# Lance0218/Pytorch-DistributedDataParallel-Training-Tricks

Measured on AMD Instinct MI355X. Metric: images/sec, higher is better.
Workload: dtype bf16; 1 GPU; model=Toy_Net, dataset=MNIST(synthetic), global_batch=1024, per_gpu_batch=1024, parallelism=dp1, optimizer=FusedSGD(momentum=0.9,nesterov)+Lookahead(k=10,a=0.5)

## Files before the change

### ddp_tricks_amd/ops/hip/bindings.cpp

```cpp
#include <torch/extension.h>

void multi_tensor_unscale(std::vector<at::Tensor> grads, at::Tensor found_inf,
                          double inv_scale,
                          c10::optional<at::Tensor> partials);
void multi_tensor_sqsum(std::vector<at::Tensor> tensors, at::Tensor partials);
void norm_finalize(at::Tensor partials, long n, double max_norm,
                   c10::optional<at::Tensor> found_inf, at::Tensor out,
                   c10::optional<at::Tensor> stats);
void multi_tensor_scale(std::vector<at::Tensor> tensors, at::Tensor coef,
                        c10::optional<at::Tensor> found_inf);
long mt_chunk_elems();
void fused_sgd(std::vector<at::Tensor> params, std::vector<at::Tensor> grads,
               std::vector<at::Tensor> bufs, double lr, double momentum,
               double wd, double nesterov, c10::optional<at::Tensor> found_inf,
               c10::optional<at::Tensor> grad_scale);
void fused_lookahead(std::vector<at::Tensor> fast, std::vector<at::Tensor> slow,
                     double alpha, c10::optional<at::Tensor> found_inf);
at::Tensor cast_to_bf16(at::Tensor x);
at::Tensor pad8_channels(at::Tensor x);
at::Tensor nhwc_flatten(at::Tensor x);
at::Tensor nhwc_unflatten(at::Tensor dy, long C, long H, long W);
std::vector<at::Tensor> pack_conv_weight(at::Tensor w, bool pad8,
                                         bool want_wt2);

// ... 42 lines not shown
                                           at::Tensor beta,
                                           at::Tensor running_mean,
                                           at::Tensor running_var,
                                           double momentum, double eps,
                                           c10::optional<at::Tensor> pre_stats);
std::vector<at::Tensor> bn_bwd_pool2(at::Tensor x, at::Tensor dy_pooled,
                                     at::Tensor gamma, at::Tensor save_mean,
                                     at::Tensor save_invstd, at::Tensor code);
at::Tensor bn_sync_local(at::Tensor x, c10::optional<at::Tensor> pre_stats);
std::vector<at::Tensor> bn_sync_fwd(at::Tensor x, at::Tensor gathered,
                                    at::Tensor gamma, at::Tensor beta,
                                    at::Tensor running_mean,
                                    at::Tensor running_var, double momentum,
                                    double eps, bool fuse_relu,
                                    c10::optional<at::Tensor> residual);
at::Tensor bn_sync_bwd_local(at::Tensor x, at::Tensor dy,
                             at::Tensor save_mean, at::Tensor save_invstd,
                             at::Tensor mask, bool fuse_relu);
std::vector<at::Tensor> bn_sync_bwd_dx(at::Tensor x, at::Tensor dy,
                                       at::Tensor gamma, at::Tensor save_mean,
                                       at::Tensor save_invstd, at::Tensor mask,
                                       bool fuse_relu, at::Tensor gathered,
                                       at::Tensor count, bool want_dresid);

at::Tensor gemm_tn(at::Tensor A, at::Tensor B, c10::optional<at::Tensor> bias,
                   bool out_f32);
at::Tensor transpose_bf16(at::Tensor x);
at::Tensor col_sum(at::Tensor x);
at::Tensor linear_fwd(at::Tensor x, at::Tensor w, c10::optional<at::Tensor> bias);
at::Tensor linear_dgrad(at::Tensor dy, at::Tensor w);
at::Tensor linear_wgrad(at::Tensor dy, at::Tensor x);

at::Tensor conv2d_fwd(at::Tensor x, at::Tensor w, c10::optional<at::Tensor> bias,
                      long stride, long pad);
std::vector<at::Tensor> conv2d_fwd_stats(at::Tensor x, at::Tensor w,
                                         c10::optional<at::Tensor> bias,
                                         long stride, long pad);
at::Tensor conv2d_dgrad(at::Tensor dy, at::Tensor wt2, long N, long C, long H,
                        long W, long R, long S, long stride, long pad,
                        c10::optional<at::Tensor> addend, long group);
std::tuple<std::string, long, long, long> conv2d_dgrad_plan(
    long N, long C, long H, long W, long Ko, long R, long S, long stride,
    long pad, long group);
std::vector<at::Tensor> conv2d_dgrad_bn(at::Tensor dy, at::Tensor wt2,
                                        long N, long C, long H, long W,
                                        long R, long S, long pad,
                                        at::Tensor bn_x, at::Tensor bn_mask,
                                        at::Tensor bn_mean,
                                        at::Tensor bn_invstd);
at::Tensor conv2d_wgrad(at::Tensor dy, at::Tensor x, long R, long S,
                        long stride, long pad);
std::vector<at::Tensor> conv2d_wgrad_bias(at::Tensor dy, at::Tensor x,
                                          long R, long S, long stride,
                                          long pad);
std::tuple<std::string, long, bool> conv2d_wgrad_plan(
    long N, long C, long H, long W, long Ko, long R, long S, long stride,
    long pad, bool want_bias);

std::vector<at::Tensor> batch_gather_aug(at::Tensor store, at::Tensor labels,
                                         at::Tensor index, at::Tensor lut,
                                         long pad, bool hflip, long seed,
                                         long epoch);
std::vector<at::Tensor> batch_gather_cutmix(at::Tensor store, at::Tensor labels,
                                            at::Tensor index, at::Tensor lut,
                                            long pad, bool hflip, long seed,
                                            long epoch, long prob_thresh);

void register_comm(py::module_& m);

PYBIND11_MODULE(TORCH_EXTENSION_NAME, m) {
    register_comm(m);
    m.def("multi_tensor_unscale", &multi_tensor_unscale,
          "fused unscale + inf check over grad tensors; with partials also "
// ... 71 lines not shown
    m.def("bn_bwd_pool2", &bn_bwd_pool2,
          py::arg("x"), py::arg("dy_pooled"), py::arg("gamma"),
          py::arg("save_mean"), py::arg("save_invstd"), py::arg("code"));
    m.def("bn_sync_local", &bn_sync_local,
          "SyncBatchNorm forward, rank-local half: [sum | sumsq | count] row",
          py::arg("x"), py::arg("pre_stats") = c10::nullopt);
    m.def("bn_sync_fwd", &bn_sync_fwd,
          "SyncBatchNorm forward, cross-rank half over gathered rows",
          py::arg("x"), py::arg("gathered"), py::arg("gamma"),
          py::arg("beta"), py::arg("running_mean"), py::arg("running_var"),
          py::arg("momentum"), py::arg("eps"), py::arg("fuse_relu") = false,
          py::arg("residual") = c10::nullopt);
    m.def("bn_sync_bwd_local", &bn_sync_bwd_local,
          "SyncBatchNorm backward, rank-local half: [dbeta | dgamma] row",
          py::arg("x"), py::arg("dy"), py::arg("save_mean"),
          py::arg("save_invstd"), py::arg("mask"),
          py::arg("fuse_relu") = false);
    m.def("bn_sync_bwd_dx", &bn_sync_bwd_dx,
          "SyncBatchNorm backward, cross-rank half over gathered rows",
          py::arg("x"), py::arg("dy"), py::arg("gamma"), py::arg("save_mean"),
          py::arg("save_invstd"), py::arg("mask"), py::arg("fuse_relu"),
          py::arg("gathered"), py::arg("count"),
          py::arg("want_dresid") = false);
    m.def("gemm_tn", &gemm_tn, py::arg("A"), py::arg("B"),
          py::arg("bias") = c10::nullopt, py::arg("out_f32") = false);
    m.def("transpose_bf16", &transpose_bf16);
    m.def("col_sum", &col_sum);
    m.def("linear_fwd", &linear_fwd, py::arg("x"), py::arg("w"),
          py::arg("bias") = c10::nullopt);
    m.def("linear_dgrad", &linear_dgrad);
    m.def("linear_wgrad", &linear_wgrad);
    m.def("conv2d_fwd", &conv2d_fwd, py::arg("x"), py::arg("w"),
          py::arg("bias") = c10::nullopt, py::arg("stride") = 1,
          py::arg("pad") = 0);
    m.def("conv2d_fwd_stats", &conv2d_fwd_stats, py::arg("x"), py::arg("w"),
          py::arg("bias") = c10::nullopt, py::arg("stride") = 1,
          py::arg("pad") = 0);
    m.def("conv2d_dgrad", &conv2d_dgrad,
          py::arg("dy"), py::arg("wt2"), py::arg("N"), py::arg("C"),
          py::arg("H"), py::arg("W"), py::arg("R"), py::arg("S"),
          py::arg("stride"), py::arg("pad"),
          py::arg("addend") = c10::nullopt, py::arg("group") = -1);
    m.def("conv2d_dgrad_plan", &conv2d_dgrad_plan,
          "(name, G, k_tiles_issued, k_tiles_raster) conv2d_dgrad would run "
          "for this shape; group -1 automatic, 0 raster, 32/64/128 forces "
          "that tap-uniform group size; launches nothing",
          py::arg("N"), py::arg("C"), py::arg("H"), py::arg("W"),
          py::arg("Ko"), py::arg("R"), py::arg("S"), py::arg("stride"),
          py::arg("pad"), py::arg("group") = -1);
    m.def("conv2d_dgrad_bn", &conv2d_dgrad_bn);
    m.def("conv2d_wgrad", &conv2d_wgrad);
    m.def("conv2d_wgrad_bias", &conv2d_wgrad_bias);
    m.def("conv2d_wgrad_plan", &conv2d_wgrad_plan,
          "(leaf name, split, fused_bias) conv2d_wgrad[_bias] would run for "
          "this shape under this process's DDPX_WGRAD_V; launches nothing",
          py::arg("N"), py::arg("C"), py::arg("H"), py::arg("W"),
          py::arg("Ko"), py::arg("R"), py::arg("S"), py::arg("stride"),
          py::arg("pad"), py::arg("want_bias"));
    m.def("batch_gather_aug", &batch_gather_aug,
          "uint8 HWC device store -> (bf16 channels_last batch, labels): "
          "gather by index + crop/flip + LUT normalise in one launch",
          py::arg("store"), py::arg("labels"), py::arg("index"),
          py::arg("lut"), py::arg("pad"), py::arg("hflip"), py::arg("seed"),
          py::arg("epoch"));
    m.def("batch_gather_cutmix", &batch_gather_cutmix,
          "batch_gather_aug with CutMix: (images, labels_a, labels_b, lam); "
          "prob_thresh is the apply probability in 1/65536",
          py::arg("store"), py::arg("labels"), py::arg("index"),
          py::arg("lut"), py::arg("pad"), py::arg("hflip"), py::arg("seed"),
          py::arg("epoch"), py::arg("prob_thresh"));
}
```

### ddp_tricks_amd/ops/hip/conv.hip

```cpp

#include <torch/extension.h>
#include <ATen/hip/HIPContext.h>
#include <climits>
#include <string>
#include <tuple>
#include "common.h"

typedef short bf16x8_t __attribute__((ext_vector_type(8)));

constexpr int CBM = 128, CBK = 64;

struct ConvShape {
    int N, H, W, C;
    int Ko, R, S;
    int P, Q;
    int stride, pad;
    FastDiv fdQ, fdP, fdW, fdH, fdC, fdS, fdKo;
    int cls_a, cls_b, nr, ns;
    int taps_r[4], taps_s[4];
    int off_r[4], off_s[4];
    int Hfull, Wfull;
    FastDiv fdNs;
    FastDiv fdGHW;
    int lgG;
};

static inline void init_fastdiv(ConvShape& cs) {
    cs.fdQ.init(cs.Q); cs.fdP.init(cs.P); cs.fdW.init(cs.W);
    cs.fdH.init(cs.H); cs.fdC.init(cs.C); cs.fdS.init(cs.S);
    cs.fdKo.init(cs.Ko);
    cs.fdGHW.init(1); cs.lgG = 0;
}

__host__ __device__ inline unsigned dgrad_tap_mask(
        int m_first, int m_last, int GHW, int lgG, int H, int W, int P, int Q,
        int R, int S, int pad) {
    const int g0 = m_first / GHW, g1 = m_last / GHW;
    int pix0 = 0, pix1 = H * W - 1;
    if (g0 == g1) {
        pix0 = (m_first - g0 * GHW) >> lgG;
        pix1 = (m_last - g0 * GHW) >> lgG;
    }
    const int h0 = pix0 / W, h1 = pix1 / W;
    unsigned mask = 0;
    for (int h = h0; h <= h1; ++h) {
        const int wa = h == h0 ? pix0 - h0 * W : 0;
        const int wb = h == h1 ? pix1 - h1 * W : W - 1;
        const int ra = h + pad - P + 1 > 0 ? h + pad - P + 1 : 0;
        const int rb = h + pad < R - 1 ? h + pad : R - 1;
        const int sa = wa + pad - Q + 1 > 0 ? wa + pad - Q + 1 : 0;
        const int sb = wb + pad < S - 1 ? wb + pad : S - 1;
        for (int r = ra; r <= rb; ++r)
            for (int sx = sa; sx <= sb; ++sx)
                mask |= 1u << (r * S + sx);
    }
    return mask;
}


__device__ __align__(16) unsigned char g_zero16[16];

struct BnFuse {
    const bf16* x;
    const unsigned char* mask;
    const float* mean;
    const float* invstd;
    float* slab;
};

template <int MODE, int TBN, int WAVES_M, int WAVES_N, bool STRIDE1,
          int CBM_T, bool TAPS = false>
__device__ __forceinline__
void conv_gemm_body(const bf16* __restrict__ Asrc,
                    const bf16* __restrict__ Bsrc,
                    const float* __restrict__ bias, bf16* __restrict__ out,
                    const ConvShape& cs, int M, int Kgemm, int Nout,
                    float* __restrict__ stats, BnFuse bn,
                    const bf16* __restrict__ addin) {
    constexpr int WM = CBM_T / WAVES_M;
    constexpr int WN = TBN / WAVES_N;
    constexpr int MI = WM / 16;
    constexpr int NI = WN / 16;
    constexpr int A_CHUNKS = CBM_T / 8;
    constexpr int B_CHUNKS = TBN / 8;
    __shared__ bf16 lds_a[1][CBM_T][CBK];
    __shared__ bf16 lds_b[1][TBN][CBK];
    static_assert(!TAPS || (MODE == 1 && STRIDE1), "TAPS is stride-1 dgrad");
    const int tile_m = TAPS && (gridDim.x & 7) == 0
        ? (int)(blockIdx.x & 7) * (int)(gridDim.x >> 3) + (int)(blockIdx.x >> 3)
        : (int)blockIdx.x;
    const int m0 = tile_m * CBM_T;
    const int n0 = blockIdx.y * TBN;
    const int tid = threadIdx.x;
    const int lane = tid & 63;
    const int wid = tid >> 6;
    const int wr = wid / WAVES_N, wc = wid % WAVES_N;

    f32x4 acc[MI][NI] = {};
    const int pl_row = lane >> 3;
    const int pl_segp = lane & 7;

    constexpr int A_PER = A_CHUNKS / 4;
    long ri_nb[A_PER];
    int ri_u[A_PER], ri_v[A_PER];
    #pragma unroll
    for (int ci = 0; ci < A_PER; ++ci) {
        const int ch = wid + ci * 4;
        const int row = ch * 8 + pl_row;
        const int gm = m0 + row;
        ri_u[ci] = INT_MIN;
        if (gm < M) {
            if (MODE == 0) {
                unsigned rem = fd_div(gm, cs.fdQ);
                int q = fd_mod(gm, cs.fdQ, rem);
                unsigned n = fd_div(rem, cs.fdP);
                int p = fd_mod(rem, cs.fdP, n);
                ri_nb[ci] = (long)n * cs.H;
                ri_u[ci] = p * cs.stride - cs.pad;
                ri_v[ci] = q * cs.stride - cs.pad;
            } else if (MODE == 2) {
                unsigned rem = fd_div(gm, cs.fdW);
                int w1 = fd_mod(gm, cs.fdW, rem);
                unsigned n = fd_div(rem, cs.fdH);
                int h1 = fd_mod(rem, cs.fdH, n);
                ri_nb[ci] = (long)n * cs.P;
                ri_u[ci] = h1;
                ri_v[ci] = w1;
            } else if (TAPS) {
                unsigned grp = fd_div(gm, cs.fdGHW);
                unsigned rem = fd_mod(gm, cs.fdGHW, grp);
                unsigned pix = rem >> cs.lgG;
                unsigned n = (grp << cs.lgG) + (rem & ((1u << cs.lgG) - 1));
                unsigned h = fd_div(pix, cs.fdW);
                int wcol = fd_mod(pix, cs.fdW, h);
                ri_nb[ci] = (long)n * cs.P;
                ri_u[ci] = (int)h + cs.pad;
                ri_v[ci] = wcol + cs.pad;
            } else {
                unsigned rem = fd_div(gm, cs.fdW);
                int wcol = fd_mod(gm, cs.fdW, rem);
                unsigned n = fd_div(rem, cs.fdH);
                int h = fd_mod(rem, cs.fdH, n);
                ri_nb[ci] = (long)n * cs.P;
                ri_u[ci] = h + cs.pad;
                ri_v[ci] = wcol + cs.pad;
            }
        }
    }

    auto issue_tile = [&](int kt, int buf) {
        #pragma unroll
        for (int ci = 0; ci < A_PER; ++ci) {
            const int ch = wid + ci * 4;
            int row = ch * 8 + pl_row;
            int seg = pl_segp ^ (row & 7);
            int gk = kt + seg * 8;
            const bf16* src = reinterpret_cast<const bf16*>(g_zero16);
            if (ri_u[ci] != INT_MIN && gk < Kgemm) {
                if (MODE == 0) {
                    unsigned rs = fd_div(gk, cs.fdC);
                    int c = fd_mod(gk, cs.fdC, rs);
                    int r = fd_div(rs, cs.fdS);
                    int sx = fd_mod(rs, cs.fdS, r);
                    int h = ri_u[ci] + r;
                    int wcol = ri_v[ci] + sx;
                    if (h >= 0 && h < cs.H && wcol >= 0 && wcol < cs.W)
                        src = &Asrc[((ri_nb[ci] + h) * cs.W + wcol) * cs.C + c];
                } else if (MODE == 2) {
                    unsigned rs2 = fd_div(gk, cs.fdKo);
                    int ko = fd_mod(gk, cs.fdKo, rs2);
                    int ti = fd_div(rs2, cs.fdNs);
                    int si = fd_mod(rs2, cs.fdNs, ti);
                    int p = ri_u[ci] + cs.off_r[ti];
                    int q = ri_v[ci] + cs.off_s[si];
                    if (p >= 0 && p < cs.P && q >= 0 && q < cs.Q)
                        src = &Asrc[((ri_nb[ci] + p) * cs.Q + q) * cs.Ko + ko];
                } else if (STRIDE1) {
                    unsigned rs = fd_div(gk, cs.fdKo);
                    int ko = fd_mod(gk, cs.fdKo, rs);
                    int r = fd_div(rs, cs.fdS);
                    int sx = fd_mod(rs, cs.fdS, r);
// ... 19 lines not shown
                (__attribute__((address_space(3))) unsigned short*)&lds_a[buf][ch * 8][0],
                16, 0, 0);
        }
        for (int ch = wid; ch < B_CHUNKS; ch += 4) {
            int row = ch * 8 + pl_row;
            int seg = pl_segp ^ (row & 7);
            int gn = n0 + row, gk = kt + seg * 8;
            const bf16* src = reinterpret_cast<const bf16*>(g_zero16);
            if (MODE == 2) {
                if (gn < Nout && gk < Kgemm) {
                    unsigned rs2 = fd_div(gk, cs.fdKo);
                    int ko = fd_mod(gk, cs.fdKo, rs2);
                    int ri = fd_div(rs2, cs.fdNs);
                    int si = fd_mod(rs2, cs.fdNs, ri);
                    long gk_full = ((long)cs.taps_r[ri] * cs.S
                                    + cs.taps_s[si]) * cs.Ko + ko;
                    src = &Bsrc[(long)gn * (cs.R * cs.S * cs.Ko) + gk_full];
                }
            } else if (gn < Nout && gk < Kgemm)
                src = &Bsrc[(long)gn * Kgemm + gk];
            __builtin_amdgcn_global_load_lds(
                (const __attribute__((address_space(1))) unsigned short*)src,
                (__attribute__((address_space(3))) unsigned short*)&lds_b[buf][ch * 8][0],
                16, 0, 0);
        }
    };

    constexpr int buf = 0;
    unsigned tap_mask = 0;
    if (TAPS)
        tap_mask = __builtin_amdgcn_readfirstlane(dgrad_tap_mask(
            m0, min(m0 + CBM_T, M) - 1, (int)cs.fdGHW.d, cs.lgG, cs.H, cs.W,
            cs.P, cs.Q, cs.R, cs.S, cs.pad));
    int tap = 0, tap_end = cs.Ko;
    for (int kt = 0; kt < Kgemm; kt += CBK) {
        if (TAPS) {
            if (kt == tap_end) { ++tap; tap_end += cs.Ko; }
            if (!((tap_mask >> tap) & 1u)) { kt = tap_end - CBK; continue; }
        }
        issue_tile(kt, 0);
        __syncthreads();
        #pragma unroll
        for (int ks = 0; ks < CBK; ks += 32) {
            bf16x8_t af[MI], bfr[NI];
            const int kgrp = (ks >> 3) + (lane >> 4);
            #pragma unroll
            for (int mi = 0; mi < MI; ++mi) {
                int row = wr * WM + mi * 16 + (lane & 15);
                af[mi] = *reinterpret_cast<const bf16x8_t*>(
                    &lds_a[buf][row][(kgrp ^ (row & 7)) * 8]);
            }
            #pragma unroll
            for (int ni = 0; ni < NI; ++ni) {
                int row = wc * WN + ni * 16 + (lane & 15);
                bfr[ni] = *reinterpret_cast<const bf16x8_t*>(
                    &lds_b[buf][row][(kgrp ^ (row & 7)) * 8]);
            }
            #pragma unroll
            for (int mi = 0; mi < MI; ++mi)
                #pragma unroll
                for (int ni = 0; ni < NI; ++ni)
                    acc[mi][ni] = __builtin_amdgcn_mfma_f32_16x16x32_bf16(
                        af[mi], bfr[ni], acc[mi][ni], 0, 0, 0);
        }
        __syncthreads();
    }

    float psum[NI] = {}, psq[NI] = {};
    #pragma unroll
    for (int mi = 0; mi < MI; ++mi)
        #pragma unroll
        for (int ni = 0; ni < NI; ++ni) {
            int col = n0 + wc * WN + ni * 16 + (lane & 15);
            if (col >= Nout) continue;
            float badd = bias ? bias[col] : 0.f;
            #pragma unroll
            for (int r = 0; r < 4; ++r) {
                int row = m0 + wr * WM + mi * 16 + (lane >> 4) * 4 + r;
                if (row >= M) continue;
                if (MODE == 0 && stats) {
                    float v = acc[mi][ni][r] + badd;
                    psum[ni] += v;
                    psq[ni] = fmaf(v, v, psq[ni]);
                }
                if (MODE == 2) {
                    unsigned rem = fd_div(row, cs.fdW);
                    int w1 = fd_mod(row, cs.fdW, rem);
                    unsigned n = fd_div(rem, cs.fdH);
                    int h1 = fd_mod(rem, cs.fdH, n);
                    long addr = (((long)n * cs.Hfull + cs.cls_a
                                  + (long)h1 * cs.stride) * cs.Wfull
                                 + cs.cls_b + (long)w1 * cs.stride) * Nout
                                + col;
                    out[addr] = f2bf(acc[mi][ni][r] + badd);
                }
            }
        }

// ... 106 lines not shown
        float* red = reinterpret_cast<float*>(&lds_a[0][0][0]);
        #pragma unroll
        for (int ni = 0; ni < NI; ++ni) {
            float a = psum[ni], b = psq[ni];
            a += __shfl_down(a, 32, 64);
            a += __shfl_down(a, 16, 64);
            b += __shfl_down(b, 32, 64);
            b += __shfl_down(b, 16, 64);
            if ((lane & 48) == 0) {
                int cl = wc * WN + ni * 16 + (lane & 15);
                red[(wr * TBN + cl) * 2] = a;
                red[(wr * TBN + cl) * 2 + 1] = b;
            }
        }
        __syncthreads();
        const int gridM = gridDim.x;
        for (int cl = tid; cl < TBN; cl += 256) {
            float a = 0.f, b = 0.f;
            #pragma unroll
            for (int w = 0; w < WAVES_M; ++w) {
                a += red[(w * TBN + cl) * 2];
                b += red[(w * TBN + cl) * 2 + 1];
            }
            int col = n0 + cl;
            if (col < Nout) {
                stats[(long)col * gridM + blockIdx.x] = a;
                stats[(long)Nout * gridM + (long)col * gridM + blockIdx.x] = b;
            }
        }
    }
}

template <int MODE, int TBN, int WAVES_M, int WAVES_N, bool STRIDE1 = true,
          int CBM_T = CBM, bool TAPS = false>
__global__ __launch_bounds__(256, 4)
void k_conv_gemm(const bf16* __restrict__ Asrc, const bf16* __restrict__ Bsrc,
                 const float* __restrict__ bias, bf16* __restrict__ out,
                 ConvShape cs, int M, int Kgemm, int Nout,
                 float* __restrict__ stats = nullptr,
                 BnFuse bn = BnFuse{},
                 const bf16* __restrict__ addin = nullptr) {
    conv_gemm_body<MODE, TBN, WAVES_M, WAVES_N, STRIDE1, CBM_T, TAPS>(
        Asrc, Bsrc, bias, out, cs, M, Kgemm, Nout, stats, bn, addin);
}


struct ClsPack {
    ConvShape cs[4];
    int M[4];
    int K[4];
};

template <int TBN, int WAVES_M, int WAVES_N>
__global__ __launch_bounds__(256, 4)
void k_conv_gemm_cls(const bf16* __restrict__ Asrc,
                     const bf16* __restrict__ Bsrc, bf16* __restrict__ out,
                     ClsPack pack, int Nout) {
    const int z = blockIdx.z;
    const int M = pack.M[z];
    if ((int)blockIdx.x * CBM >= M) return;
    conv_gemm_body<2, TBN, WAVES_M, WAVES_N, true, CBM>(
        Asrc, Bsrc, nullptr, out, pack.cs[z], M, pack.K[z], Nout,
        nullptr, BnFuse{}, nullptr);
}

__global__ void k_conv_small_cin(const bf16* __restrict__ x,
                                 const bf16* __restrict__ w,
                                 const float* __restrict__ bias,
                                 bf16* __restrict__ y, ConvShape cs, long M) {
    extern __shared__ __attribute__((aligned(16))) char smem[];
    bf16* wlds = reinterpret_cast<bf16*>(smem);
    int rsc = cs.R * cs.S * cs.C;
    for (int i = threadIdx.x; i < cs.Ko * rsc; i += blockDim.x)
        wlds[i] = w[i];
    __syncthreads();
// ... 780 lines not shown
    int ko = i % cs.Ko;
    int rc = i / cs.Ko;
    float v = 0.f;
    for (int s = 0; s < S; ++s)
        v += slab[((long)s * rsc_total + rc) * cs.Ko + ko];
    int c = rc % cs.C, rs = rc / cs.C;
    dw[((long)ko * cs.C + c) * (cs.R * cs.S) + rs] = v;
}


static ConvShape make_shape(int N, int C, int H, int W, int Ko, int R, int S,
                            int stride, int pad) {
    ConvShape cs;
    cs.N = N; cs.C = C; cs.H = H; cs.W = W;
    cs.Ko = Ko; cs.R = R; cs.S = S; cs.stride = stride; cs.pad = pad;
    cs.P = (cs.H + 2 * pad - R) / stride + 1;
    cs.Q = (cs.W + 2 * pad - S) / stride + 1;
    init_fastdiv(cs);
    return cs;
}

static ConvShape make_shape(const at::Tensor& x, int Ko, int R, int S,
                            int stride, int pad) {
    return make_shape(x.size(0), x.size(1), x.size(2), x.size(3), Ko, R, S,
                      stride, pad);
}

static at::Tensor empty_nhwc(const at::Tensor& like, long n, long c, long h,
                             long w) {
    return at::empty({n, c, h, w},
                     like.options().memory_format(at::MemoryFormat::ChannelsLast));
}

template <int MODE, bool STRIDE1 = true>
static void launch_conv_gemm(hipStream_t stream, int grid_m, int n_channels,
                             bool narrow, const bf16* Asrc, const bf16* Bsrc,
                             const float* bias, bf16* out,
                             const ConvShape& cs, long M, int Kgemm,
                             float* stats, BnFuse bn, const bf16* addin) {
    if (n_channels >= 128 && !narrow)
        hipLaunchKernelGGL((k_conv_gemm<MODE, 128, 2, 2, STRIDE1>),
                           dim3(grid_m, ceil_div_i(n_channels, 128)),
                           dim3(256), 0, stream, Asrc, Bsrc, bias, out, cs,
                           (int)M, Kgemm, n_channels, stats, bn, addin);
    else
        hipLaunchKernelGGL((k_conv_gemm<MODE, 64, 4, 1, STRIDE1>),
                           dim3(grid_m, ceil_div_i(n_channels, 64)),
                           dim3(256), 0, stream, Asrc, Bsrc, bias, out, cs,
                           (int)M, Kgemm, n_channels, stats, bn, addin);
    HIP_CHECK_LAST();
}

static void launch_conv_gemm_cls(hipStream_t stream, int grid_m,
                                 int n_channels, int ncls, const bf16* Asrc,
                                 const bf16* Bsrc, bf16* out,
                                 const ClsPack& pack) {
    if (n_channels >= 128)
        hipLaunchKernelGGL((k_conv_gemm_cls<128, 2, 2>),
                           dim3(grid_m, ceil_div_i(n_channels, 128), ncls),
                           dim3(256), 0, stream, Asrc, Bsrc, out, pack,
                           n_channels);
    else
        hipLaunchKernelGGL((k_conv_gemm_cls<64, 4, 1>),
                           dim3(grid_m, ceil_div_i(n_channels, 64), ncls),
                           dim3(256), 0, stream, Asrc, Bsrc, out, pack,
                           n_channels);
    HIP_CHECK_LAST();
}

static std::vector<at::Tensor> conv_fwd_impl(
        const at::Tensor& x, const at::Tensor& w,
        const c10::optional<at::Tensor>& bias, long stride, long pad,
        bool want_stats) {
    TORCH_CHECK(x.is_cuda() && x.scalar_type() == at::kBFloat16);
    ConvShape cs = make_shape(x, w.size(0), w.size(2), w.size(3),
                              (int)stride, (int)pad);
    int Kgemm = cs.R * cs.S * cs.C;
    long M = (long)cs.N * cs.P * cs.Q;
    auto stream = at::hip::getCurrentHIPStream();
    const float* bp = bias.has_value() ? bias->data_ptr<float>() : nullptr;
    const bf16* xp = reinterpret_cast<const bf16*>(x.data_ptr());
    const bf16* wp = reinterpret_cast<const bf16*>(w.data_ptr());
    auto y = empty_nhwc(x, cs.N, cs.Ko, cs.P, cs.Q);
    bf16* yp = reinterpret_cast<bf16*>(y.data_ptr());

    if (cs.C < 8 && !want_stats) {
        TORCH_CHECK(cs.Ko % 8 == 0);
        int lds = cs.Ko * Kgemm * 2;
        long total = M * (cs.Ko / 8);
        int blocks = std::min<long>(8192, ceil_div_i(total, 256));
        hipLaunchKernelGGL(k_conv_small_cin, dim3(blocks), dim3(256), lds,
                           stream.stream(), xp, wp, bp, yp, cs, M);
        HIP_CHECK_LAST();
        return {y, at::Tensor()};
    }
    TORCH_CHECK(cs.C % 8 == 0, want_stats
                ? "stats path needs the MFMA conv (C%8==0)"
                : "conv fwd needs C % 8 == 0");
    TORCH_CHECK(cs.Ko % 8 == 0, "conv fwd needs Ko % 8 == 0");
    const int gridM = ceil_div_i(M, CBM);
    at::Tensor slab;
    if (want_stats)
        slab = at::empty({2, (long)cs.Ko, (long)gridM},
                         x.options().dtype(at::kFloat));
    static const char* tbn_env = getenv("DDPX_CONV_TBN64");
    launch_conv_gemm<0>(stream.stream(), gridM, cs.Ko,
                        tbn_env && !want_stats, xp, wp, bp, yp, cs, M, Kgemm,
                        want_stats ? slab.data_ptr<float>() : nullptr,
                        BnFuse{}, nullptr);
    return {y, slab};
}

at::Tensor conv2d_fwd(at::Tensor x, at::Tensor w,
                      c10::optional<at::Tensor> bias, long stride, long pad) {
    return conv_fwd_impl(x, w, bias, stride, pad, false)[0];
}

std::vector<at::Tensor> conv2d_fwd_stats(at::Tensor x, at::Tensor w,
                                         c10::optional<at::Tensor> bias,
                                         long stride, long pad) {
    return conv_fwd_impl(x, w, bias, stride, pad, true);
}

static ConvShape dgrad_shape(const at::Tensor& dy, long N, long C, long H,
                             long W, long R, long S, long stride, long pad) {
    ConvShape cs;
    cs.N = N; cs.C = C; cs.H = H; cs.W = W;
    cs.Ko = dy.size(1); cs.P = dy.size(2); cs.Q = dy.size(3);
    cs.R = R; cs.S = S; cs.stride = stride; cs.pad = pad;
    init_fastdiv(cs);
    TORCH_CHECK(cs.Ko % 8 == 0, "conv dgrad needs Ko % 8 == 0");
    TORCH_CHECK(cs.C % 8 == 0, "conv dgrad needs C % 8 == 0");
    return cs;
}

struct DgradPlan {
    const char* name;
    int G;
    long k_tiles, k_tiles_raster;
};

static DgradPlan plan_dgrad(const ConvShape& cs, bool want_bn, long group) {
    TORCH_CHECK(group == -1 || group == 0 || group == 32 || group == 64 ||
                group == 128, "conv dgrad group must be -1 (automatic), 0 "
                "(raster), 32, 64 or 128; got ", group);
    const long M = (long)cs.N * cs.H * cs.W;
    const int tiles = ceil_div_i(M, CBM);
    DgradPlan p{"raster", 0, 0, 0};
    p.k_tiles_raster = (long)tiles * ceil_div_i((long)cs.R * cs.S * cs.Ko, CBK);
    p.k_tiles = p.k_tiles_raster;
    const bool fits = cs.stride == 1 && cs.Ko % CBK == 0 &&
                      cs.R * cs.S <= 32 && !want_bn && M < INT_MAX;
    if (!fits || group == 0) return p;

// ... 6 lines not shown
        long n = 0;
        for (int t = 0; t < walk; ++t) {
            const int m0 = t * CBM;
            const int m1 = (int)std::min<long>(m0 + CBM, M) - 1;
            n += __builtin_popcount(dgrad_tap_mask(
                m0, m1, (int)ghw, lg, cs.H, cs.W, cs.P, cs.Q, cs.R, cs.S,
                cs.pad));
        }
        if (periodic) n *= cs.N / G;
        return n * (cs.Ko / CBK);
    };
    static const struct { int C, H, W, Ko, R, S, pad, G; } MEASURED[] = {
        {128, 12, 12, 256, 3, 3, 0, 128},
        {256, 10, 10, 512, 3, 3, 0, 128},
    };
    int G = (int)std::max<long>(group, 0);
    if (group < 0 && cs.N >= 1024)
        for (const auto& m : MEASURED)
            if (cs.C == m.C && cs.H == m.H && cs.W == m.W && cs.Ko == m.Ko &&
                cs.R == m.R && cs.S == m.S && cs.pad == m.pad)
                G = m.G;
    if (G == 0 || cs.N % G != 0) return p;
    const long issued = count(G);
    if (issued >= p.k_tiles_raster) return p;
    p.name = "taps";
    p.G = G;
    p.k_tiles = issued;
    return p;
}

static at::Tensor dgrad_stride1(const at::Tensor& dy, const at::Tensor& wt2,
                                ConvShape cs,
                                const c10::optional<at::Tensor>& addend,
                                BnFuse bn, long group) {
    auto dx = empty_nhwc(dy, cs.N, cs.C, cs.H, cs.W);
    const bf16* adp = nullptr;
    if (addend.has_value()) {
        TORCH_CHECK(addend->sizes() == dx.sizes() &&
                    addend->scalar_type() == at::kBFloat16);
        adp = reinterpret_cast<const bf16*>(addend->data_ptr());
    }
    const long M = (long)cs.N * cs.H * cs.W;
    const int grid_m = ceil_div_i(M, CBM);
    const int Kgemm = cs.R * cs.S * cs.Ko;
    auto stream = at::hip::getCurrentHIPStream().stream();
    const bf16* dyp = reinterpret_cast<const bf16*>(dy.data_ptr());
    const bf16* wtp = reinterpret_cast<const bf16*>(wt2.data_ptr());
    bf16* dxp = reinterpret_cast<bf16*>(dx.data_ptr());
    const DgradPlan plan = plan_dgrad(cs, bn.slab != nullptr, group);
    if (plan.G == 0) {
        launch_conv_gemm<1>(stream, grid_m, cs.C, false, dyp, wtp, nullptr,
                            dxp, cs, M, Kgemm, nullptr, bn, adp);
        return dx;
    }
    cs.fdGHW.init((unsigned)plan.G * cs.H * cs.W);
    cs.lgG = 0;
    while ((1 << cs.lgG) < plan.G) ++cs.lgG;
    if (cs.C >= 128)
        hipLaunchKernelGGL((k_conv_gemm<1, 128, 2, 2, true, CBM, true>),
                           dim3(grid_m, ceil_div_i(cs.C, 128)), dim3(256), 0,
                           stream, dyp, wtp, nullptr, dxp, cs, (int)M, Kgemm,
                           cs.C, nullptr, BnFuse{}, adp);
    else
        hipLaunchKernelGGL((k_conv_gemm<1, 64, 4, 1, true, CBM, true>),
                           dim3(grid_m, ceil_div_i(cs.C, 64)), dim3(256), 0,
                           stream, dyp, wtp, nullptr, dxp, cs, (int)M, Kgemm,
                           cs.C, nullptr, BnFuse{}, adp);
    HIP_CHECK_LAST();
    return dx;
}

at::Tensor conv2d_dgrad(at::Tensor dy, at::Tensor wt2, long N, long C,
                        long H, long W, long R, long S, long stride, long pad,
                        c10::optional<at::Tensor> addend, long group) {
    ConvShape cs = dgrad_shape(dy, N, C, H, W, R, S, stride, pad);
    TORCH_CHECK(!addend.has_value() || cs.stride == 1,
                "fused dgrad addend needs stride 1");
    if (cs.stride == 1)
        return dgrad_stride1(dy, wt2, cs, addend, BnFuse{}, group);
    plan_dgrad(cs, false, group);

    auto dx = empty_nhwc(dy, cs.N, cs.C, cs.H, cs.W);
    auto stream = at::hip::getCurrentHIPStream();
    const bf16* dyp_ = reinterpret_cast<const bf16*>(dy.data_ptr());
    const bf16* wt2p = reinterpret_cast<const bf16*>(wt2.data_ptr());
    bf16* dxp = reinterpret_cast<bf16*>(dx.data_ptr());
    const int st = cs.stride;
    {
        bool any_empty = false;
        for (int a = 0; a < st && !any_empty; ++a) {
            int nr = 0;
            for (int r = 0; r < cs.R; ++r)
                if (((a + cs.pad - r) % st + st) % st == 0) ++nr;
            if (nr == 0) any_empty = true;
        }
        if (!any_empty)
            for (int b = 0; b < st && !any_empty; ++b) {
                int ns = 0;
                for (int sidx = 0; sidx < cs.S; ++sidx)
                    if (((b + cs.pad - sidx) % st + st) % st == 0) ++ns;
                if (ns == 0) any_empty = true;
            }
        if (any_empty) dx.zero_();
    }
    ClsPack pack{};
    int ncls = 0;
    int maxTiles = 0;
    for (int a = 0; a < st; ++a) {
        for (int b = 0; b < st; ++b) {
            ConvShape c2 = cs;
            c2.cls_a = a; c2.cls_b = b;
            c2.Hfull = cs.H; c2.Wfull = cs.W;
            c2.nr = 0; c2.ns = 0;
// ... 23 lines not shown
                pack.K[ncls] = K2;
                maxTiles = std::max(maxTiles, (int)ceil_div_i(M2, CBM));
                ++ncls;
            } else {
                launch_conv_gemm<2>(stream.stream(), ceil_div_i(M2, CBM),
                                    cs.C, false, dyp_, wt2p, nullptr, dxp,
                                    c2, M2, K2, nullptr, BnFuse{}, nullptr);
            }
        }
    }
    if (ncls > 0)
        launch_conv_gemm_cls(stream.stream(), maxTiles, cs.C, ncls, dyp_,
                             wt2p, dxp, pack);
    return dx;
}

std::vector<at::Tensor> conv2d_dgrad_bn(at::Tensor dy, at::Tensor wt2,
                                        long N, long C, long H, long W,
                                        long R, long S, long pad,
                                        at::Tensor bn_x, at::Tensor bn_mask,
                                        at::Tensor bn_mean,
                                        at::Tensor bn_invstd) {
    ConvShape cs = dgrad_shape(dy, N, C, H, W, R, S, 1, pad);
    const int gridM = ceil_div_i((long)cs.N * cs.H * cs.W, CBM);
    auto slab = at::empty({2, (long)cs.C, (long)gridM},
                          dy.options().dtype(at::kFloat));
    BnFuse bn;
    bn.x = reinterpret_cast<const bf16*>(bn_x.data_ptr());
    bn.mask = bn_mask.numel()
        ? bn_mask.data_ptr<unsigned char>() : nullptr;
    bn.mean = bn_mean.data_ptr<float>();
    bn.invstd = bn_invstd.data_ptr<float>();
    bn.slab = slab.data_ptr<float>();
    return {dgrad_stride1(dy, wt2, cs, c10::nullopt, bn, -1), slab};
}

std::tuple<std::string, long, long, long> conv2d_dgrad_plan(
        long N, long C, long H, long W, long Ko, long R, long S, long stride,
        long pad, long group) {
    TORCH_CHECK(N > 0 && C > 0 && Ko > 0 && R > 0 && S > 0 && stride > 0 &&
                pad >= 0 && H + 2 * pad >= R && W + 2 * pad >= S);
    ConvShape cs = make_shape((int)N, (int)C, (int)H, (int)W, (int)Ko, (int)R,
                              (int)S, (int)stride, (int)pad);
    const DgradPlan p = plan_dgrad(cs, false, group);
    return std::make_tuple(std::string(p.name), (long)p.G, p.k_tiles,
                           p.k_tiles_raster);
}

at::Tensor col_sum(at::Tensor x);


enum class WgradLeaf {
    StemStream, C1R3, SmallRsc, SmallCin,
    SbPair32, SbPair64,
    WidePair32, WidePair64, WideDma32, WideDma64,
};

using WgradMfmaKernel = void (*)(const bf16*, const bf16*, float*, ConvShape,
                                 long, int, int);
static const struct { const char* name; WgradMfmaKernel kern[2]; }
WGRAD_LEAVES[] = {
    {"c1_r3_stream", {}}, {"c1_r3", {}}, {"small_rsc", {}}, {"small_cin", {}},
    {"sb_pair<32>", {k_conv_wgrad_sb_pair<32>, k_conv_wgrad_sb_pair<32>}},
    {"sb_pair<64>", {k_conv_wgrad_sb_pair<64>, k_conv_wgrad_sb_pair<64>}},
    {"wide_pair<32>", {k_conv_wgrad_wide_pair<32, false>,
                       k_conv_wgrad_wide_pair<32, true>}},
    {"wide_pair<64>", {k_conv_wgrad_wide_pair<64, false>,
                       k_conv_wgrad_wide_pair<64, true>}},
    {"wide_dma<32>", {k_conv_wgrad_wide_dma<32, false>,
                      k_conv_wgrad_wide_dma<32, true>}},
    {"wide_dma<64>", {k_conv_wgrad_wide_dma<64, false>,
                      k_conv_wgrad_wide_dma<64, true>}},
};
static_assert(sizeof(WGRAD_LEAVES) / sizeof(WGRAD_LEAVES[0]) ==
              (int)WgradLeaf::WideDma64 + 1, "one row per WgradLeaf");

struct WgradPlan {
    WgradLeaf leaf;
    int S;
// ... 210 lines not shown
```

Before: 403,400 images/sec.

## Add tap-walk K loop for conv forward and stride-1 dgrad

Adds a WALK variant of the conv implicit-GEMM body. When channels are a multiple of the K tile, the K loop iterates over filter taps (r, s) and channel chunks directly, using precomputed per-row base offsets and wave-uniform addresses. This avoids the per-tile division-based index decode in the K loop. It also specialises the no-padding forward case to skip bounds checks, and dispatches automatically when the shape fits, overridable through a new kwalk argument. The cost is extra kernel instantiations and higher register use for the per-row offsets.

```diff
diff --git a/ddp_tricks_amd/ops/hip/bindings.cpp b/ddp_tricks_amd/ops/hip/bindings.cpp
--- a/ddp_tricks_amd/ops/hip/bindings.cpp
+++ b/ddp_tricks_amd/ops/hip/bindings.cpp
@@ -98,13 +98,17 @@
 at::Tensor linear_wgrad(at::Tensor dy, at::Tensor x);
 
 at::Tensor conv2d_fwd(at::Tensor x, at::Tensor w, c10::optional<at::Tensor> bias,
-                      long stride, long pad);
+                      long stride, long pad, long kwalk);
 std::vector<at::Tensor> conv2d_fwd_stats(at::Tensor x, at::Tensor w,
                                          c10::optional<at::Tensor> bias,
-                                         long stride, long pad);
+                                         long stride, long pad, long kwalk);
 at::Tensor conv2d_dgrad(at::Tensor dy, at::Tensor wt2, long N, long C, long H,
                         long W, long R, long S, long stride, long pad,
-                        c10::optional<at::Tensor> addend, long group);
+                        c10::optional<at::Tensor> addend, long group,
+                        long kwalk);
+std::string conv2d_kloop_plan(long mode, long N, long C, long H, long W,
+                              long Ko, long R, long S, long stride, long pad,
+                              long kwalk);
 std::tuple<std::string, long, long, long> conv2d_dgrad_plan(
     long N, long C, long H, long W, long Ko, long R, long S, long stride,
     long pad, long group);
@@ -242,15 +246,24 @@
     m.def("linear_wgrad", &linear_wgrad);
     m.def("conv2d_fwd", &conv2d_fwd, py::arg("x"), py::arg("w"),
           py::arg("bias") = c10::nullopt, py::arg("stride") = 1,
-          py::arg("pad") = 0);
+          py::arg("pad") = 0, py::arg("kwalk") = -1);
     m.def("conv2d_fwd_stats", &conv2d_fwd_stats, py::arg("x"), py::arg("w"),
           py::arg("bias") = c10::nullopt, py::arg("stride") = 1,
-          py::arg("pad") = 0);
+          py::arg("pad") = 0, py::arg("kwalk") = -1);
     m.def("conv2d_dgrad", &conv2d_dgrad,
           py::arg("dy"), py::arg("wt2"), py::arg("N"), py::arg("C"),
           py::arg("H"), py::arg("W"), py::arg("R"), py::arg("S"),
           py::arg("stride"), py::arg("pad"),
-          py::arg("addend") = c10::nullopt, py::arg("group") = -1);
+          py::arg("addend") = c10::nullopt, py::arg("group") = -1,
+          py::arg("kwalk") = -1);
+    m.def("conv2d_kloop_plan", &conv2d_kloop_plan,
+          "'walk' or 'decode': the K loop conv2d_fwd[_stats] (mode 0) or "
+          "conv2d_dgrad (mode 1) would run for this shape; kwalk -1 "
+          "automatic, 0 decode, 1 forces the scalar tap walk; launches "
+          "nothing",
+          py::arg("mode"), py::arg("N"), py::arg("C"), py::arg("H"),
+          py::arg("W"), py::arg("Ko"), py::arg("R"), py::arg("S"),
+          py::arg("stride"), py::arg("pad"), py::arg("kwalk") = -1);
     m.def("conv2d_dgrad_plan", &conv2d_dgrad_plan,
           "(name, G, k_tiles_issued, k_tiles_raster) conv2d_dgrad would run "
           "for this shape; group -1 automatic, 0 raster, 32/64/128 forces "
diff --git a/ddp_tricks_amd/ops/hip/conv.hip b/ddp_tricks_amd/ops/hip/conv.hip
--- a/ddp_tricks_amd/ops/hip/conv.hip
+++ b/ddp_tricks_amd/ops/hip/conv.hip
@@ -4,6 +4,7 @@
 #include <climits>
 #include <string>
 #include <tuple>
+#include <type_traits>
 #include "common.h"
 
 typedef short bf16x8_t __attribute__((ext_vector_type(8)));
@@ -69,7 +70,7 @@
 };
 
 template <int MODE, int TBN, int WAVES_M, int WAVES_N, bool STRIDE1,
-          int CBM_T, bool TAPS = false>
+          int CBM_T, bool TAPS = false, bool WALK = false>
 __device__ __forceinline__
 void conv_gemm_body(const bf16* __restrict__ Asrc,
                     const bf16* __restrict__ Bsrc,
@@ -86,6 +87,8 @@
     __shared__ bf16 lds_a[1][CBM_T][CBK];
     __shared__ bf16 lds_b[1][TBN][CBK];
     static_assert(!TAPS || (MODE == 1 && STRIDE1), "TAPS is stride-1 dgrad");
+    static_assert(!WALK || MODE == 0 || (MODE == 1 && STRIDE1),
+                  "WALK is forward or stride-1 dgrad");
     const int tile_m = TAPS && (gridDim.x & 7) == 0
         ? (int)(blockIdx.x & 7) * (int)(gridDim.x >> 3) + (int)(blockIdx.x >> 3)
         : (int)blockIdx.x;
@@ -103,12 +106,17 @@
     constexpr int A_PER = A_CHUNKS / 4;
     long ri_nb[A_PER];
     int ri_u[A_PER], ri_v[A_PER];
+    long a_off[A_PER];
+    bool a_rv[A_PER];
+    const int walk_seg8 = (pl_segp ^ pl_row) * 8;
+    const int widu = WALK ? __builtin_amdgcn_readfirstlane(wid) : wid;
     #pragma unroll
     for (int ci = 0; ci < A_PER; ++ci) {
         const int ch = wid + ci * 4;
         const int row = ch * 8 + pl_row;
         const int gm = m0 + row;
         ri_u[ci] = INT_MIN;
+        if (WALK) { ri_v[ci] = 0; a_off[ci] = 0; a_rv[ci] = false; }
         if (gm < M) {
             if (MODE == 0) {
                 unsigned rem = fd_div(gm, cs.fdQ);
@@ -145,8 +153,70 @@
                 ri_u[ci] = h + cs.pad;
                 ri_v[ci] = wcol + cs.pad;
             }
-        }
-    }
+            if (WALK) {
+                a_rv[ci] = true;
+                a_off[ci] = (((ri_nb[ci] + ri_u[ci]) * (MODE == 0 ? cs.W : cs.Q)
+                              + ri_v[ci]) * (MODE == 0 ? cs.C : cs.Ko)
+                             + walk_seg8) * (long)sizeof(bf16);
+            }
+        }
+    }
+    constexpr int B_PER = B_CHUNKS / 4;
+    long b_off = 0;
+    bool b_cv[B_PER];
+    if (WALK) {
+        b_off = ((long)(n0 + widu * 8 + pl_row) * Kgemm + walk_seg8)
+                * (long)sizeof(bf16);
+        #pragma unroll
+        for (int bi = 0; bi < B_PER; ++bi)
+            b_cv[bi] = n0 + (widu + bi * 4) * 8 + pl_row < Nout;
+    }
+    unsigned long zaddr = reinterpret_cast<unsigned long>(g_zero16);
+    if (WALK) asm volatile("" : "+s"(zaddr));
+
+    auto issue_tile_walk = [&](int kt, int r, int sx, int c0, auto nopad_c) {
+        constexpr bool NOPAD = decltype(nopad_c)::value;
+        const int tap_off = MODE == 0 ? (r * cs.W + sx) * cs.C + c0
+                                      : c0 - (r * cs.Q + sx) * cs.Ko;
+        const unsigned long abase = reinterpret_cast<unsigned long>(Asrc)
+            + (unsigned long)((long)tap_off * (long)sizeof(bf16));
+        #pragma unroll
+        for (int ci = 0; ci < A_PER; ++ci) {
+            bool ok;
+            if (NOPAD)
+                ok = a_rv[ci];
+            else if (MODE == 0)
+                ok = (unsigned)ri_u[ci] + (unsigned)r < (unsigned)cs.H &&
+                     (unsigned)ri_v[ci] + (unsigned)sx < (unsigned)cs.W;
+            else
+                ok = (unsigned)ri_u[ci] - (unsigned)r < (unsigned)cs.P &&
+                     (unsigned)ri_v[ci] - (unsigned)sx < (unsigned)cs.Q;
+            const unsigned long addr =
+                ok ? abase + (unsigned long)a_off[ci] : zaddr;
+            __builtin_amdgcn_global_load_lds(
+                reinterpret_cast<const __attribute__((address_space(1)))
+                                 unsigned short*>(addr),
+                (__attribute__((address_space(3))) unsigned short*)
+                    &lds_a[0][(widu + ci * 4) * 8][0],
+                16, 0, 0);
+        }
+        const unsigned long bbase = reinterpret_cast<unsigned long>(Bsrc)
+            + (unsigned long)((long)kt * (long)sizeof(bf16));
+        #pragma unroll
+        for (int bi = 0; bi < B_PER; ++bi) {
+            const unsigned long addr = b_cv[bi]
+                ? bbase + (unsigned long)((long)bi * 32 * Kgemm
+                                          * (long)sizeof(bf16))
+                      + (unsigned long)b_off
+                : zaddr;
+            __builtin_amdgcn_global_load_lds(
+                reinterpret_cast<const __attribute__((address_space(1)))
+                                 unsigned short*>(addr),
+                (__attribute__((address_space(3))) unsigned short*)
+                    &lds_b[0][(widu + bi * 4) * 8][0],
+                16, 0, 0);
+        }
+    };
 
     auto issue_tile = [&](int kt, int buf) {
         #pragma unroll
@@ -232,13 +302,7 @@
         tap_mask = __builtin_amdgcn_readfirstlane(dgrad_tap_mask(
             m0, min(m0 + CBM_T, M) - 1, (int)cs.fdGHW.d, cs.lgG, cs.H, cs.W,
             cs.P, cs.Q, cs.R, cs.S, cs.pad));
-    int tap = 0, tap_end = cs.Ko;
-    for (int kt = 0; kt < Kgemm; kt += CBK) {
-        if (TAPS) {
-            if (kt == tap_end) { ++tap; tap_end += cs.Ko; }
-            if (!((tap_mask >> tap) & 1u)) { kt = tap_end - CBK; continue; }
-        }
-        issue_tile(kt, 0);
+    auto mma_tile = [&]() {
         __syncthreads();
         #pragma unroll
         for (int ks = 0; ks < CBK; ks += 32) {
@@ -264,6 +328,32 @@
                         af[mi], bfr[ni], acc[mi][ni], 0, 0, 0);
         }
         __syncthreads();
+    };
+    auto walk_loop = [&](auto nopad_c) {
+        const int Cd = MODE == 0 ? cs.C : cs.Ko;
+        int kt = 0, tap = 0;
+        for (int r = 0; r < cs.R; ++r)
+            for (int sx = 0; sx < cs.S; ++sx, ++tap, kt += Cd) {
+                if (TAPS && !((tap_mask >> tap) & 1u)) continue;
+                for (int c0 = 0; c0 < Cd; c0 += CBK) {
+                    issue_tile_walk(kt + c0, r, sx, c0, nopad_c);
+                    mma_tile();
+                }
+            }
+    };
+    if (WALK) {
+        if (MODE == 0 && cs.pad == 0) walk_loop(std::true_type{});
+        else walk_loop(std::false_type{});
+    } else {
+        int tap = 0, tap_end = cs.Ko;
+        for (int kt = 0; kt < Kgemm; kt += CBK) {
+            if (TAPS) {
+                if (kt == tap_end) { ++tap; tap_end += cs.Ko; }
+                if (!((tap_mask >> tap) & 1u)) { kt = tap_end - CBK; continue; }
+            }
+            issue_tile(kt, 0);
+            mma_tile();
+        }
     }
 
     float psum[NI] = {}, psq[NI] = {};
@@ -436,7 +526,7 @@
 }
 
 template <int MODE, int TBN, int WAVES_M, int WAVES_N, bool STRIDE1 = true,
-          int CBM_T = CBM, bool TAPS = false>
+          int CBM_T = CBM, bool TAPS = false, bool WALK = false>
 __global__ __launch_bounds__(256, 4)
 void k_conv_gemm(const bf16* __restrict__ Asrc, const bf16* __restrict__ Bsrc,
                  const float* __restrict__ bias, bf16* __restrict__ out,
@@ -444,7 +534,7 @@
                  float* __restrict__ stats = nullptr,
                  BnFuse bn = BnFuse{},
                  const bf16* __restrict__ addin = nullptr) {
-    conv_gemm_body<MODE, TBN, WAVES_M, WAVES_N, STRIDE1, CBM_T, TAPS>(
+    conv_gemm_body<MODE, TBN, WAVES_M, WAVES_N, STRIDE1, CBM_T, TAPS, WALK>(
         Asrc, Bsrc, bias, out, cs, M, Kgemm, Nout, stats, bn, addin);
 }
 
@@ -1291,12 +1381,45 @@
                      like.options().memory_format(at::MemoryFormat::ChannelsLast));
 }
 
+static const char* plan_kloop(int mode, const ConvShape& cs, long kwalk) {
+    TORCH_CHECK(kwalk >= -1 && kwalk <= 1, "conv kwalk must be -1 "
+                "(automatic), 0 (decode) or 1 (walk); got ", kwalk);
+    bool fits = false;
+    if (mode == 0)
+        fits = cs.C % CBK == 0 &&
+               ((long)cs.R * cs.W + cs.S) * cs.C < INT_MAX;
+    else if (mode == 1)
+        fits = cs.stride == 1 && cs.Ko % CBK == 0 &&
+               ((long)cs.R * cs.Q + cs.S) * cs.Ko < INT_MAX;
+    if (!fits || kwalk == 0) return "decode";
+    return "walk";
+}
+
 template <int MODE, bool STRIDE1 = true>
 static void launch_conv_gemm(hipStream_t stream, int grid_m, int n_channels,
                              bool narrow, const bf16* Asrc, const bf16* Bsrc,
                              const float* bias, bf16* out,
                              const ConvShape& cs, long M, int Kgemm,
-                             float* stats, BnFuse bn, const bf16* addin) {
+                             float* stats, BnFuse bn, const bf16* addin,
+                             long kwalk = 0) {
+    if constexpr (MODE != 2) {
+        if (plan_kloop(MODE, cs, kwalk)[0] == 'w') {
+            if (n_channels >= 128 && !narrow)
+                hipLaunchKernelGGL(
+                    (k_conv_gemm<MODE, 128, 2, 2, STRIDE1, CBM, false, true>),
+                    dim3(grid_m, ceil_div_i(n_channels, 128)), dim3(256), 0,
+                    stream, Asrc, Bsrc, bias, out, cs, (int)M, Kgemm,
+                    n_channels, stats, bn, addin);
+            else
+                hipLaunchKernelGGL(
+                    (k_conv_gemm<MODE, 64, 4, 1, STRIDE1, CBM, false, true>),
+                    dim3(grid_m, ceil_div_i(n_channels, 64)), dim3(256), 0,
+                    stream, Asrc, Bsrc, bias, out, cs, (int)M, Kgemm,
+                    n_channels, stats, bn, addin);
+            HIP_CHECK_LAST();
+            return;
+        }
+    }
     if (n_channels >= 128 && !narrow)
         hipLaunchKernelGGL((k_conv_gemm<MODE, 128, 2, 2, STRIDE1>),
                            dim3(grid_m, ceil_div_i(n_channels, 128)),
@@ -1330,7 +1453,7 @@
 static std::vector<at::Tensor> conv_fwd_impl(
         const at::Tensor& x, const at::Tensor& w,
         const c10::optional<at::Tensor>& bias, long stride, long pad,
-        bool want_stats) {
+        bool want_stats, long kwalk) {
     TORCH_CHECK(x.is_cuda() && x.scalar_type() == at::kBFloat16);
     ConvShape cs = make_shape(x, w.size(0), w.size(2), w.size(3),
                               (int)stride, (int)pad);
@@ -1344,6 +1467,7 @@
     bf16* yp = reinterpret_cast<bf16*>(y.data_ptr());
 
     if (cs.C < 8 && !want_stats) {
+        plan_kloop(0, cs, kwalk);
         TORCH_CHECK(cs.Ko % 8 == 0);
         int lds = cs.Ko * Kgemm * 2;
         long total = M * (cs.Ko / 8);
@@ -1366,19 +1490,20 @@
     launch_conv_gemm<0>(stream.stream(), gridM, cs.Ko,
                         tbn_env && !want_stats, xp, wp, bp, yp, cs, M, Kgemm,
                         want_stats ? slab.data_ptr<float>() : nullptr,
-                        BnFuse{}, nullptr);
+                        BnFuse{}, nullptr, kwalk);
     return {y, slab};
 }
 
 at::Tensor conv2d_fwd(at::Tensor x, at::Tensor w,
-                      c10::optional<at::Tensor> bias, long stride, long pad) {
-    return conv_fwd_impl(x, w, bias, stride, pad, false)[0];
+                      c10::optional<at::Tensor> bias, long stride, long pad,
+                      long kwalk) {
+    return conv_fwd_impl(x, w, bias, stride, pad, false, kwalk)[0];
 }
 
 std::vector<at::Tensor> conv2d_fwd_stats(at::Tensor x, at::Tensor w,
                                          c10::optional<at::Tensor> bias,
-                                         long stride, long pad) {
-    return conv_fwd_impl(x, w, bias, stride, pad, true);
+                                         long stride, long pad, long kwalk) {
+    return conv_fwd_impl(x, w, bias, stride, pad, true, kwalk);
 }
 
 static ConvShape dgrad_shape(const at::Tensor& dy, long N, long C, long H,
@@ -1451,7 +1576,7 @@
 static at::Tensor dgrad_stride1(const at::Tensor& dy, const at::Tensor& wt2,
                                 ConvShape cs,
                                 const c10::optional<at::Tensor>& addend,
-                                BnFuse bn, long group) {
+                                BnFuse bn, long group, long kwalk) {
     auto dx = empty_nhwc(dy, cs.N, cs.C, cs.H, cs.W);
     const bf16* adp = nullptr;
     if (addend.has_value()) {
@@ -1469,35 +1594,41 @@
     const DgradPlan plan = plan_dgrad(cs, bn.slab != nullptr, group);
     if (plan.G == 0) {
         launch_conv_gemm<1>(stream, grid_m, cs.C, false, dyp, wtp, nullptr,
-                            dxp, cs, M, Kgemm, nullptr, bn, adp);
+                            dxp, cs, M, Kgemm, nullptr, bn, adp, kwalk);
         return dx;
     }
     cs.fdGHW.init((unsigned)plan.G * cs.H * cs.W);
     cs.lgG = 0;
     while ((1 << cs.lgG) < plan.G) ++cs.lgG;
-    if (cs.C >= 128)
-        hipLaunchKernelGGL((k_conv_gemm<1, 128, 2, 2, true, CBM, true>),
-                           dim3(grid_m, ceil_div_i(cs.C, 128)), dim3(256), 0,
-                           stream, dyp, wtp, nullptr, dxp, cs, (int)M, Kgemm,
-                           cs.C, nullptr, BnFuse{}, adp);
-    else
-        hipLaunchKernelGGL((k_conv_gemm<1, 64, 4, 1, true, CBM, true>),
-                           dim3(grid_m, ceil_div_i(cs.C, 64)), dim3(256), 0,
-                           stream, dyp, wtp, nullptr, dxp, cs, (int)M, Kgemm,
-                           cs.C, nullptr, BnFuse{}, adp);
+    const bool walk = plan_kloop(1, cs, kwalk)[0] == 'w';
+    const dim3 grid(grid_m, ceil_div_i(cs.C, cs.C >= 128 ? 128 : 64));
+    auto launch = [&](auto kern) {
+        hipLaunchKernelGGL(kern, grid, dim3(256), 0, stream, dyp, wtp,
+                           (const float*)nullptr, dxp, cs, (int)M, Kgemm,
+                           cs.C, (float*)nullptr, BnFuse{}, adp);
+    };
+    if (cs.C >= 128) {
+        if (walk) launch(k_conv_gemm<1, 128, 2, 2, true, CBM, true, true>);
+        else launch(k_conv_gemm<1, 128, 2, 2, true, CBM, true, false>);
+    } else {
+        if (walk) launch(k_conv_gemm<1, 64, 4, 1, true, CBM, true, true>);
+        else launch(k_conv_gemm<1, 64, 4, 1, true, CBM, true, false>);
+    }
     HIP_CHECK_LAST();
     return dx;
 }
 
 at::Tensor conv2d_dgrad(at::Tensor dy, at::Tensor wt2, long N, long C,
                         long H, long W, long R, long S, long stride, long pad,
-                        c10::optional<at::Tensor> addend, long group) {
+                        c10::optional<at::Tensor> addend, long group,
+                        long kwalk) {
     ConvShape cs = dgrad_shape(dy, N, C, H, W, R, S, stride, pad);
     TORCH_CHECK(!addend.has_value() || cs.stride == 1,
                 "fused dgrad addend needs stride 1");
     if (cs.stride == 1)
-        return dgrad_stride1(dy, wt2, cs, addend, BnFuse{}, group);
+        return dgrad_stride1(dy, wt2, cs, addend, BnFuse{}, group, kwalk);
     plan_dgrad(cs, false, group);
+    plan_kloop(1, cs, kwalk);
 
     auto dx = empty_nhwc(dy, cs.N, cs.C, cs.H, cs.W);
     auto stream = at::hip::getCurrentHIPStream();
@@ -1587,7 +1718,7 @@
     bn.mean = bn_mean.data_ptr<float>();
     bn.invstd = bn_invstd.data_ptr<float>();
     bn.slab = slab.data_ptr<float>();
-    return {dgrad_stride1(dy, wt2, cs, c10::nullopt, bn, -1), slab};
+    return {dgrad_stride1(dy, wt2, cs, c10::nullopt, bn, -1, -1), slab};
 }
 
 std::tuple<std::string, long, long, long> conv2d_dgrad_plan(
@@ -1600,6 +1731,17 @@
     const DgradPlan p = plan_dgrad(cs, false, group);
     return std::make_tuple(std::string(p.name), (long)p.G, p.k_tiles,
                            p.k_tiles_raster);
+}
+
+std::string conv2d_kloop_plan(long mode, long N, long C, long H, long W,
+                              long Ko, long R, long S, long stride, long pad,
+                              long kwalk) {
+    TORCH_CHECK(mode == 0 || mode == 1, "mode is 0 (forward) or 1 (dgrad)");
+    TORCH_CHECK(N > 0 && C > 0 && Ko > 0 && R > 0 && S > 0 && stride > 0 &&
+                pad >= 0 && H + 2 * pad >= R && W + 2 * pad >= S);
+    ConvShape cs = make_shape((int)N, (int)C, (int)H, (int)W, (int)Ko, (int)R,
+                              (int)S, (int)stride, (int)pad);
+    return plan_kloop((int)mode, cs, kwalk);
 }
 
 at::Tensor col_sum(at::Tensor x);
```

After: 435,400 images/sec, median of 6. 7.9% higher.
